# skhu101/HumanLiff

Measured on AMD Instinct MI355X. Metric: denoise-steps/sec, higher is better.
Workload: dtype f32; 1 GPU; configs[1]: 256x256x27 tri-plane UNet (controlnet, 497M params), 1000-step DDPM p_sample_loop, batch=4 per GPU; global_batch=4, parallelism=replicas x1 (subjects sharded, final all-gather only)

## Files before the change

### humanliff_amd/_lib.py

```python
import contextlib
import ctypes as C
import os

import torch

_HERE = os.path.dirname(os.path.abspath(__file__))
LIB_PATH = os.environ.get("HL_LIB_PATH") or os.path.join(_HERE, "libhumanliff_hip.so")

HL_RENDER_MLP_FP16 = 16
HL_RENDER_MLP_BF16X3 = 32
HL_RENDER_MLP_FP16X2 = 64
HL_RENDER_FOUR_LAUNCH = 128
HL_CONV_FP32 = 0
HL_CONV_BF16X3 = 1
HL_CONV_FP32_F23 = 3
HL_CONV_FP32_DIRECT = 2
HL_CONV_BF16 = 4
HL_CONV_FP16 = 5
HL_CONV_FP32_MFMA = 6
HL_RENDER_WHITE_BKGD = 1
HL_RENDER_NORMALIZE_DEPTH = 2
HL_RENDER_REEVALUATE = 4
HL_RENDER_CLAMP_DEPTH = 8
HL_COMPOSITE_SERIAL_RAW = 1
# ... 74 lines not shown
    "hl_render_composite_backward_plan": (_i, [_i, _i]),
    "hl_render_mlp_bwd_packed_bytes": (_sz, []),
    "hl_render_mlp_pack_bwd": (_i, [C.POINTER(RenderMlpParams), _p, _p]),
    "hl_render_train_rows": (None, [C.POINTER(C.c_int), C.POINTER(C.c_int)]),
    "hl_render_eval_acts": (_i, [_p, _p, _i, _i, _p, _p, _p, _p, _p, _p, _i, _i64, _i, _p, _p, _i64, _i64, _p]),
    "hl_render_composite_backward_scratch_bytes": (_sz, [_i64, _i, _i]),
    "hl_render_composite_backward": (_i, [_p, _p, _p, _p, _p, _p, _p, _p, _p, _i64, _i, _i, _u, _p, _p, _p, _i64, _p, _p]),
    "hl_render_eval_points_acts": (_i, [_p, _p, _i, _i, _p, _p, _p, _i64, _i, _p, _p, _i64, _i64, _p]),
    "hl_render_plane_grads_points_scratch_bytes": (_sz, [_i64, _i, _i]),
    "hl_render_plane_grads_points": (_i, [_i, _i, _p, _p, _p, _i64, _i, _i, _p, _i64, _p, _p, _p]),
    "hl_render_weight_grads": (_i, [_p, _i64, _p, _i64, _i64, C.POINTER(RenderMlpParams), _p, _p]),
    "hl_render_weight_grads_scratch_bytes": (_sz, [_i64]),
    "hl_render_plane_grads_scratch_bytes": (_sz, [_i64]),
    "hl_render_mlp_backward": (_i, [_p, _p, _i, _i, _p, _p, _p, _p, _p, _p, _i, _i64, _i, _p, _p, _i64, _i64, _p, _i64, _i64, _p]),
    "hl_render_plane_grads": (_i, [_i, _i, _p, _p, _p, _p, _p, _p, _p, _i, _i64, _i, _i, _p, _i64, _p, _p, _p]),
    "hl_render_fine": (_i, [_p, _p, _i, _i, _p, _p, _p, _p, _p, _p, _i, _i64, _i, _u, _p, _p, _p, _p]),
    "hl_unet_packed_bytes": (_sz, [C.POINTER(UNetCfg)]),
    "hl_unet_create": (_i, [C.POINTER(UNetCfg), _i, C.POINTER(C.c_char_p), C.POINTER(C.c_void_p), C.POINTER(C.c_int64),
                            _p, _p, C.POINTER(C.c_void_p)]),
    "hl_unet_destroy": (None, [_p]),
    "hl_unet_workspace_bytes": (_sz, [_p, _i, _i, _i]),
    "hl_unet_forward": (_i, [_p, _p, _p, _p, _p, _p, _p, _i, _i, _i, _p, _p]),
    "hl_unet_set_overlap": (_i, [_p, _i]),
    "hl_unet_set_conv_mode": (_i, [_p, _i]),
    "hl_unet_profile": (_i, [_p, _i]),
    "hl_unet_profile_read": (_i, [_p, C.POINTER(C.c_double), C.POINTER(C.c_double), C.POINTER(C.c_int64)]),
    "hl_unet_profile_read_ex": (_i, [_p, C.POINTER(C.c_double), C.POINTER(C.c_double), C.POINTER(C.c_double), C.POINTER(C.c_int64)]),
    "hl_unet_dispatch_census": (_i, [_p, C.POINTER(C.c_int64)]),
    "hl_unet_dispatch_census_ex": (_i, [_p, _p, _i]),
    "hl_unet_profile_dominant": (_i, [_p, C.POINTER(C.c_double), C.POINTER(C.c_int)]),
    "hl_diffusion_step": (_i, [_i, _p, _p, _p, _p, _p, _p, _p, _i64, _i, _i, _i, _p, _p]),
    "hl_diffusion_q_sample": (_i, [_p, _p, _p, _p, _p, _i64, _i, _i, _p]),
    "hl_diffusion_reverse_step": (_i, [_i, _p, _p, _p, _p, _p, _p, _i64, _i, _i, _i, _p]),
    "hl_diffusion_vb_scratch_bytes": (_sz, [_i64, _i]),
    "hl_diffusion_vb_terms": (_i, [_i, _i, _i, _p, _p, _p, _p, _p, _i64, _p, _p, _i64, _i, _i, _p, _p, _p, _i64, _i64, _p, _sz, _p]),
    "hl_diffusion_prior_bpd": (_i, [_p, _p, _i64, _i, _i, _p, _p, _sz, _p]),
    "hl_conv2d_scratch_bytes": (_sz, [_i] * 10),
    "hl_conv2d_plan": (_i, [_i] * 10 + [C.POINTER(C.c_int), C.POINTER(C.c_int)]),
    "hl_conv2d_plan_ex": (_i, [_i] * 12 + [C.POINTER(C.c_int)]),
    "hl_conv2d_gn_scratch_bytes": (_sz, [_i] * 10),
    "hl_conv2d_bwd_data_scratch_bytes": (_sz, [_i] * 11),
    "hl_conv2d_nhwc": (_i, [_p, _i, _i, _i, _i, _p, _p, _i, _i, _i, _i, _p, _p, _i, _p, _p, _p, _sz, _p]),
    "hl_conv2d_nhwc_mode": (_i, [_i, _p, _i, _i, _i, _i, _p, _p, _i, _i, _i, _i, _p, _p, _i, _p, _p, _p, _sz, _p]),
    "hl_conv2d_nhwc_gn": (_i, [_i, _p, _i, _i, _i, _i, _p, _p, _i, _i, _i, _i, _p, _p, _i, _p, _p, _p, _p, _p, _p, C.POINTER(C.c_int), _p, _sz, _p]),
    "hl_conv2d_bwd_data_plan": (_i, [_i] * 11 + [C.POINTER(C.c_int), C.POINTER(C.c_int)]),
    "hl_conv2d_nhwc_bwd_data": (_i, [_i, _p, _i, _i, _i, _i, _p, _i, _i, _i, _i, _i, _p, _i, _p, _sz, _p]),
# ... 165 lines not shown
```

### humanliff_amd/csrc/hl_unet.cpp

```cpp
#include <cstdint>
#include <string>
#include <unordered_map>
#include <utility>
#include <vector>

#include "hl_stat_book.h"
#include "hl_unet_kernels.h"
#include <algorithm>

namespace {

using hl::ConvArgs;
using hl::View;

static inline int round_up(int v, int m) { return (v + m - 1) / m * m; }

using hl::WeightForm;
using hl::conv_forms;
using hl::conv_mode_known;

struct Conv {
    hl::ConvWeights w;
    const float *bias = nullptr;
    int Cin = 0, Cin_pad = 0, Cout = 0, ks = 1;
};
struct Norm {
    const float *gamma = nullptr, *beta = nullptr;
    int C = 0;
    float eps = 1e-5f;
};
struct Res {
    Norm n1, n2;
    Conv c1, c2, skip;
    bool has_skip = false;
    bool aware = false;
    long emb_off = 0;
    int Cin = 0, Cout = 0;
};
struct Attn {
    Norm norm;
    Conv qkv, proj;
    int C = 0, heads = 1;
};
struct Xf {
    Norm norm;
    Conv proj_in, proj_out, qkv, out1, ff_in, ff_out;
    const float *ln1_g = nullptr, *ln1_b = nullptr, *ln3_g = nullptr, *ln3_b = nullptr;
    const float *v2_w = nullptr, *o2_w = nullptr, *o2_b = nullptr;
    int C = 0, heads = 1;
};
enum Kind { K_CONV, K_RES, K_ATTN, K_DOWN, K_UP, K_XF };
struct Layer {
    Kind kind;
    int idx;
};
struct Block {
    std::vector<Layer> layers;
    int Cout = 0;
    int ds_out = 1;
};

struct Net {
    hl_unet_cfg cfg{};
    std::unordered_map<std::string, std::pair<const float *, int64_t>> sd;
    std::vector<Conv> convs;
    std::vector<Res> res;
    std::vector<Attn> attn;
    std::vector<Xf> xf;
    std::vector<Block> in_blocks, out_blocks, cond_blocks;
    Block middle;
    std::vector<int> proj_cond;
    Conv out_conv;
    Norm out_norm;
    const float *te0_w = nullptr, *te0_b = nullptr, *te2_w = nullptr, *te2_b = nullptr, *label = nullptr;
    Conv ada1, ada2;
    const float *ada_w = nullptr, *ada_b = nullptr;
    const float *emb_w = nullptr, *emb_b = nullptr;
    long emb_total = 0;
    int E = 0;
    int Cpad0 = 0;
    float *packed = nullptr;
    size_t packed_off = 0;
    bool dry = true;
    hipStream_t st = nullptr;
    std::string err;
    hipStream_t side = nullptr;
    hipEvent_t ev_fork = nullptr, ev_join = nullptr;
    std::vector<hipEvent_t> ev_block;
    bool overlap = true;
    int conv_mode = HL_CONV_FP32;
    bool prof = false;
    std::vector<hipEvent_t> ev_pool;
    struct Span { int cat; size_t a, b; double flops, exec; int key[5]; long mid; };
    double dom[4] = {0, 0, 0, 0};
// ... 26 lines not shown
    if (expect >= 0 && it->second.second != expect) {
        if (n.err.empty()) n.err = "shape mismatch for " + name + ": got " + std::to_string(it->second.second) + " elements, expected " + std::to_string(expect);
        return nullptr;
    }
    return it->second.first;
}

size_t form_floats(size_t bytes) { return (bytes / 4 + 63) / 64 * 64; }
size_t conv_forms_floats(int Cout, int Cin_pad, int ks) {
    size_t t = 0;
    for (int f = 0; f < hl::kWeightForms; ++f) t += form_floats(hl::conv_form_bytes((WeightForm)f, Cout, Cin_pad, ks));
    return t;
}
Conv make_conv_w(Net &n, const float *w, const float *bias, int Cin, int Cout, int ks, bool ups = false);
Conv make_conv(Net &n, const std::string &p, int Cin, int Cout, int ks, bool has_bias = true, bool ups = false) {
    const float *w = lookup(n, p + ".weight", (int64_t)Cout * Cin * ks * ks);
    const float *b = has_bias ? lookup(n, p + ".bias", Cout) : nullptr;
    return make_conv_w(n, w, b, Cin, Cout, ks, ups);
}
Conv make_conv_w(Net &n, const float *w, const float *bias, int Cin, int Cout, int ks, bool ups) {
    Conv c;
    c.Cin = Cin; c.Cin_pad = round_up(Cin, 16); c.Cout = Cout; c.ks = ks;
    c.bias = n.dry ? nullptr : bias;
    const int cp = c.Cin_pad;
    for (int f = 0; f < hl::kWeightForms; ++f) {
        const size_t bytes = hl::conv_form_bytes((WeightForm)f, Cout, cp, ks, true, ups);
        if (!bytes) continue;
        float *dst = n.dry ? nullptr : n.packed + n.packed_off;
        n.packed_off += form_floats(bytes);
        if (n.dry || !w) continue;
        c.w.p[f] = dst;
        if (hl::conv_pack_form((WeightForm)f, w, Cout, Cin, cp, ks, dst, n.st) != 0 && n.err.empty()) n.err = hl_last_error();
    }
    return c;
}
Norm make_norm(Net &n, const std::string &p, int C) {
    Norm g;
    g.C = C;
    g.gamma = lookup(n, p + ".weight", C);
    g.beta = lookup(n, p + ".bias", C);
    return g;
}

struct EmbPiece { std::string name; int O; long off; };

int add_res(Net &n, std::vector<EmbPiece> &emb, const std::string &p, int Cin, int Cout, bool aware = false) {
// ... 92 lines not shown
            ch = co;
            if (has_ds(c, ds)) {
                if (c.cross_attn) b.layers.push_back({K_XF, add_xf(n, p + ".1", ch, c.num_heads)});
                else b.layers.push_back({K_ATTN, add_attn(n, p + ".1", ch, c.num_heads)});
            }
            b.Cout = ch; b.ds_out = ds;
            blocks.push_back(b);
            chans.push_back(ch);
            ++bi;
        }
        if (level != c.n_levels - 1) {
            Block b;
            const std::string p = root + "." + std::to_string(bi);
            b.layers.push_back({K_DOWN, add_conv(n, p + ".0.op", ch, ch, 3)});
            ds *= 2;
            b.Cout = ch; b.ds_out = ds;
            blocks.push_back(b);
            chans.push_back(ch);
            ++bi;
        }
    }
}

void build(Net &n) {
    const hl_unet_cfg &c = n.cfg;
    n.E = 4 * c.model_channels;
    n.Cpad0 = round_up(c.in_channels, 16);
    n.emb_total = 0;
    n.packed_off = 0;
    n.convs.clear(); n.res.clear(); n.attn.clear(); n.xf.clear();
    n.in_blocks.clear(); n.out_blocks.clear(); n.cond_blocks.clear(); n.proj_cond.clear();
    std::vector<EmbPiece> emb;
    n.te0_w = lookup(n, "time_embed.0.weight", (int64_t)n.E * c.model_channels);
    n.te0_b = lookup(n, "time_embed.0.bias", n.E);
    n.te2_w = lookup(n, "time_embed.2.weight", (int64_t)n.E * n.E);
    n.te2_b = lookup(n, "time_embed.2.bias", n.E);
    n.label = c.num_classes > 0 ? lookup(n, "label_emb.weight", (int64_t)c.num_classes * n.E) : nullptr;
    if (c.adagn || c.cross_attn) {
        n.ada1 = make_conv(n, "conv_proj_1", c.out_channels, 6, 3);
        n.ada2 = make_conv(n, "conv_proj_2", 6, 1, 3);
        n.ada_w = lookup(n, "linear.weight", (int64_t)n.E * 4096);
        n.ada_b = lookup(n, "linear.bias", n.E);
    }

    std::vector<int> chans;
    const bool aware = c.aware3d != 0;
// ... 21 lines not shown
            int li = 0;
            b.layers.push_back({K_RES, add_res(n, emb, p + "." + std::to_string(li++), ch + skip, co, aware)});
            ch = co;
            if (has_ds(c, ds)) {
                if (c.cross_attn) b.layers.push_back({K_XF, add_xf(n, p + "." + std::to_string(li++), ch, c.num_heads)});
                else b.layers.push_back({K_ATTN, add_attn(n, p + "." + std::to_string(li++), ch, c.num_heads_upsample)});
            }
            if (level && i == c.num_res_blocks) {
                b.layers.push_back({K_UP, add_conv(n, p + "." + std::to_string(li++) + ".conv", ch, ch, 3, true)});
                ds /= 2;
            }
            b.Cout = ch; b.ds_out = ds;
            n.out_blocks.push_back(b);
            ++bi;
        }
    }
    n.out_norm = make_norm(n, "out.0", ch);
    n.out_conv = make_conv(n, "out.2", c.model_channels, c.out_channels, 3);
    if (c.controlnet) {
        std::vector<int> cch;
        build_encoder(n, emb, "input_blocks_cond", n.cond_blocks, cch, false);
        for (size_t i = 0; i < n.cond_blocks.size(); ++i)
            n.proj_cond.push_back(add_conv(n, "input_blocks_proj_cond." + std::to_string(i), cch[i], cch[i], 1));
    }
    const size_t wfl = (size_t)n.emb_total * n.E;
    if (!n.dry) {
        float *wdst = n.packed + n.packed_off, *bdst = wdst + wfl;
        for (auto &e : emb) {
            const float *w = lookup(n, e.name + ".weight", (int64_t)e.O * n.E);
            const float *b = lookup(n, e.name + ".bias", e.O);
            if (!w || !b) continue;
            hipMemcpyAsync(wdst + (size_t)e.off * n.E, w, (size_t)e.O * n.E * sizeof(float), hipMemcpyDeviceToDevice, n.st);
            hipMemcpyAsync(bdst + e.off, b, (size_t)e.O * sizeof(float), hipMemcpyDeviceToDevice, n.st);
        }
        n.emb_w = wdst; n.emb_b = bdst;
    }
    n.packed_off += (wfl + n.emb_total + 63) / 64 * 64;
}

struct Aff { float *cA = nullptr, *cB = nullptr; hl::GnSrc gn{}; };
struct ConvOpt {
    int stride = 1, ups = 0;
    Aff af{};
    int act = 0;
    const float *res = nullptr; long res_pitch = 0;
    float *out2 = nullptr; long out2_pitch = 0;
// ... 109 lines not shown
        n.census[hl::conv_census_row(pl.path)][lvl] += 1;
        span_key[0] = (int)pl.path; span_key[1] = lvl; span_key[2] = o.ups ? 1 : 0; span_key[3] = c.Cout; span_key[4] = c.ks;
        const double fl = 2.0 * (double)out.pixels() * c.Cout * c.Cin * c.ks * c.ks;
        span_end(CAT_CONV, e0, fl, fl * hl::conv_issued_factor(pl.path) * (pl.kernel == hl::ConvKernel::H2sUp ? 4.0 / 9.0 : 1.0));
    }
    Aff coef(const View &x, const Norm &g, const float *emb, bool force_arrays = false) {
        Aff af;
        af.cA = alloc((size_t)B * x.C);
        af.cB = alloc((size_t)B * x.C);
        if (!run) return af;
        const float *gt = book.totals_of(x.p, x.C, true);
        if (gt && !force_arrays && !n.prof) {
            af.cA = af.cB = nullptr;
            af.gn.gt = gt; af.gn.C = x.C; af.gn.HW = x.H * x.W;
            af.gn.gamma = g.gamma; af.gn.beta = g.beta; af.gn.emb = emb; af.gn.emb_pitch = n.emb_total; af.gn.eps = g.eps;
            return af;
        }
        const size_t e0 = span_begin();
        if (gt) ok(hl::groupnorm_coef_stats(x, gt, g.gamma, g.beta, emb, n.emb_total, af.cA, af.cB, lane->st, g.eps));
        else ok(hl::groupnorm_coef(x, g.gamma, g.beta, emb, n.emb_total, af.cA, af.cB, lane->gn_scratch, lane->st, nullptr, g.eps));
        span_end(CAT_GN, e0, 0.0);
        return af;
    }
    void res_block(const Res &r, const View &x, const View &dst) {
        const bool noss = n.cfg.no_scale_shift;
        ConvOpt o1, o2;
        o1.af = coef(x, r.n1, nullptr); o1.act = 1; o1.stats = !noss;
        View h = plain(H / dst.H, r.Cout), in2 = h;
        conv(r.c1, x, h, o1);
        if (noss && run) ok(hl::add_rowvec(h, emb_all + r.emb_off, lane->st, n.emb_total));
        const Aff a2 = coef(h, r.n2, run && !noss ? emb_all + r.emb_off : nullptr, r.aware);
        if (r.aware) {
            in2 = plain(H / dst.H, 3 * r.Cout);
            float *sums = alloc((size_t)B * 3 * (h.H + h.W / 3) * r.Cout);
            if (run) {
                const size_t e0 = span_begin();
                ok(hl::gn_apply_3d(h, a2.cA, a2.cB, sums, in2.p, lane->st));
                span_end(CAT_GN, e0, 0.0);
            }
        } else {
            o2.af = a2; o2.act = 1;
        }
        if (r.has_skip) {
            ConvOpt sk;
            sk.stats = false;
            conv(r.skip, x, dst, sk);
        }
        o2.residual(r.has_skip ? dst : x);
        conv(r.c2, in2, dst, o2);
    }
    void attn_block(const Attn &a, const View &x, const View &dst) {
        ConvOpt oq, op;
        oq.af = coef(x, a.norm, nullptr);
        oq.stats = false;
        View qkv = plain(H / x.H, 3 * a.C);
        conv(a.qkv, x, qkv, oq);
        View o = plain(H / x.H, a.C);
        float *ost = alloc_stat(hl::conv_stats_floats(B, (long)x.H * x.W));
        if (run) {
            const size_t e0 = span_begin();
            int emitted = 0;
            ok(hl::attention(qkv.p, B, x.H * x.W, a.C, a.heads, o.p, lane->st, n.conv_mode == HL_CONV_FP32, ost, &emitted));
            if (emitted) book.produced(o.p, {ost, a.C, 0}, a.C); else book.stored_without_totals(o.p);
            const double T = (double)x.H * x.W;
            span_end(CAT_ATTN, e0, 4.0 * B * T * T * a.C);
        }
        op.residual(x);
        conv(a.proj, o, dst, op);
    }
    void xf_block(const Xf &a, const View &x, const View &dst) {
        const int ds = H / x.H;
        hipStream_t st = lane->st;
// ... 126 lines not shown
                if (run && c.controlnet) book.concat_halves(cat[j].p, cat[j].C, ch, cat_st);
                ch = n.out_blocks[j].Cout;
            }
        }
        auto first_part = [&](size_t j, int C) { View v = cat[j]; v.C = C; return v; };
        const bool fork = run && c.controlnet && n.overlap && !n.prof && n.side;
        if (fork) {
            hipEventRecord(n.ev_fork, st);
            hipStreamWaitEvent(n.side, n.ev_fork, 0);
        }
        std::vector<View> hs(nb);
        View h = xin;
        for (size_t i = 0; i < nb; ++i) {
            hs[i] = plain(n.in_blocks[i].ds_out, n.in_blocks[i].Cout);
            block(n.in_blocks[i], h, hs[i]);
            if (fork) hipEventRecord(n.ev_block[i], st);
            h = hs[i];
        }
        block(n.middle, h, first_part(0, n.middle.Cout));
        if (c.controlnet) {
            if (fork) lane = &lanes[1];
            View hc = xsum;
            for (size_t i = 0; i < nb; ++i) {
                View tmp = plain(n.cond_blocks[i].ds_out, n.cond_blocks[i].Cout);
                block(n.cond_blocks[i], hc, tmp);
                View pj = plain(n.cond_blocks[i].ds_out, n.cond_blocks[i].Cout);
                const size_t j = nb - 1 - i;
                const int Ch = cat[j].C - hs[i].C;
                if (fork) hipStreamWaitEvent(n.side, n.ev_block[i], 0);
                ConvOpt zo;
                zo.out2 = run ? cat[j].p + Ch : nullptr; zo.out2_pitch = cat[j].pitch; zo.res2 = hs[i].p; zo.res2_pitch = hs[i].pitch;
                conv(n.convs[n.proj_cond[i]], tmp, pj, zo);
                hc = pj;
            }
            if (fork) {
                hipEventRecord(n.ev_join, n.side);
                lane = &lanes[0];
                hipStreamWaitEvent(st, n.ev_join, 0);
            }
        } else if (run) {
            for (size_t i = 0; i < nb; ++i) {
                const size_t j = nb - 1 - i;
                const int Ch = cat[j].C - hs[i].C;
                hipMemcpy2DAsync(cat[j].p + Ch, cat[j].pitch * sizeof(float), hs[i].p, hs[i].pitch * sizeof(float),
                                 (size_t)hs[i].C * sizeof(float), (size_t)hs[i].pixels(), hipMemcpyDeviceToDevice, st);
                book.stored_without_totals(cat[j].p + Ch);
            }
        }
        View last;
        for (size_t j = 0; j < nb; ++j) {
            View dst = (j + 1 < nb) ? first_part(j + 1, n.out_blocks[j].Cout) : plain(n.out_blocks[j].ds_out, n.out_blocks[j].Cout);
            block(n.out_blocks[j], cat[j], dst);
            last = dst;
        }
        ConvOpt oo;
// ... 61 lines not shown
        return rc;
    }
    if (n->cfg.controlnet) {
        bool okc = hipStreamCreateWithFlags(&n->side, hipStreamNonBlocking) == hipSuccess;
        okc = okc && hipEventCreateWithFlags(&n->ev_fork, hipEventDisableTiming) == hipSuccess;
        okc = okc && hipEventCreateWithFlags(&n->ev_join, hipEventDisableTiming) == hipSuccess;
        n->ev_block.assign(n->in_blocks.size(), nullptr);
        for (auto &e : n->ev_block) okc = okc && hipEventCreateWithFlags(&e, hipEventDisableTiming) == hipSuccess;
        if (!okc) {
            (void)hipGetLastError();
            if (n->side) { hipStreamDestroy(n->side); n->side = nullptr; }
        }
    }
    *handle = n;
    return HL_OK;
}

int hl_unet_set_overlap(void *handle, int enable) {
    HL_REQUIRE(handle, "hl_unet_set_overlap: null handle");
    static_cast<Net *>(handle)->overlap = enable != 0;
    return HL_OK;
}

int hl_unet_set_conv_mode(void *handle, int mode) {
    HL_REQUIRE(handle, "hl_unet_set_conv_mode: null handle");
    HL_REQUIRE(conv_mode_known(mode), "hl_unet_set_conv_mode: unknown mode %d", mode);
    static_cast<Net *>(handle)->conv_mode = mode;
    return HL_OK;
}

void hl_unet_destroy(void *handle) { delete static_cast<Net *>(handle); }

size_t hl_unet_workspace_bytes(void *handle, int B, int H, int W) {
    if (!handle || B <= 0) return 0;
    Net &n = *static_cast<Net *>(handle);
    Exec e(n, false, nullptr, nullptr, B, H, n.cfg.aware3d ? 3 * W : W);
    e.forward(nullptr, nullptr, nullptr, nullptr, nullptr, nullptr);
    WsLayout L;
    return ws_layout(e.off, e.act_need, e.stat_off, 0, &L) ? 0 : L.total;
}

int hl_unet_forward(void *handle, const float *x, const int64_t *t, const float *t_float, const float *x_cond,
                    const int64_t *y, float *out, int B, int H, int W, void *workspace, void *stream) {
    HL_REQUIRE(handle && x && (t || t_float) && out && workspace, "hl_unet_forward: null argument");
    Net &n = *static_cast<Net *>(handle);
    const int total_ds = 1 << (n.cfg.n_levels - 1);
    HL_REQUIRE(B >= 1 && B <= 16, "hl_unet_forward: batch %d outside [1,16]", B);
    HL_REQUIRE(H % total_ds == 0 && W % total_ds == 0, "hl_unet_forward: H,W must be divisible by %d", total_ds);
    HL_REQUIRE(!n.cfg.controlnet || x_cond, "hl_unet_forward: x_cond is required with cond_type='controlnet'");
    HL_REQUIRE(!(n.cfg.adagn || n.cfg.cross_attn) || (x_cond && H == 256 && W == 256),
               "hl_unet_forward: cond_type='AdaGN' / 'cross_attention' need x_cond and 256x256 inputs (Linear(64*64, ..))");
    HL_REQUIRE(n.cfg.num_classes == 0 || y, "hl_unet_forward: y is required for a class-conditional model");
    if (n.cfg.aware3d) W *= 3;
    Exec dry(n, false, nullptr, nullptr, B, H, W);
    dry.forward(nullptr, nullptr, nullptr, nullptr, nullptr, nullptr);
    char *const ws = static_cast<char *>(workspace);
    WsLayout L;
    const int lrc = ws_layout(dry.off, dry.act_need, dry.stat_off, reinterpret_cast<uintptr_t>(ws), &L);
    if (lrc) return lrc;
    Exec e(n, true, ws, (hipStream_t)stream, B, H, W);
// ... 332 lines not shown
    View v; v.p = out; v.N = N; conv_out_hw(H, W, ks, stride, upsample, &v.H, &v.W); v.C = Cout; v.pitch = Cout;
    if (h_used_stats) *h_used_stats = slots;
    if (slots > 0) {
        return hl::groupnorm_coef_stats(v, stats, gamma, beta, nullptr, 0, next_coefA, next_coefB, (hipStream_t)stream);
    }
    return hl::groupnorm_coef(v, gamma, beta, nullptr, 0, next_coefA, next_coefB, gn_scr, (hipStream_t)stream);
}

int hl_conv2d_nhwc(const float *in, int N, int H, int W, int Cin, const float *w_oihw, const float *bias, int Cout, int ks,
                   int stride, int upsample, const float *coefA, const float *coefB, int silu, const float *residual,
                   float *out, void *scratch, size_t scratch_bytes, void *stream) {
    return conv2d_single(HL_CONV_FP32_DIRECT, in, N, H, W, Cin, w_oihw, bias, Cout, ks, stride, upsample, coefA, coefB, silu, residual, out,
                         scratch, scratch_bytes, stream);
}

int hl_conv2d_nhwc_mode(int conv_mode, const float *in, int N, int H, int W, int Cin, const float *w_oihw, const float *bias,
                        int Cout, int ks, int stride, int upsample, const float *coefA, const float *coefB, int silu,
                        const float *residual, float *out, void *scratch, size_t scratch_bytes, void *stream) {
    HL_REQUIRE(conv_mode_known(conv_mode), "hl_conv2d_nhwc_mode: unknown mode %d", conv_mode);
    return conv2d_single(conv_mode, in, N, H, W, Cin, w_oihw, bias, Cout, ks, stride, upsample, coefA, coefB, silu, residual, out,
                         scratch, scratch_bytes, stream);
}

int hl_debug_set_h16_min_blocks(long v) { hl::set_h16_min_blocks(v); return HL_OK; }
int hl_debug_set_single_op_scale_source(int from_totals) { g_single_op_scale_from_totals = from_totals != 0; return HL_OK; }
int hl_debug_set_attention_tiling(int query_tiles, int placement) { return hl::debug_set_attention_tiling(query_tiles, placement); }

size_t hl_groupnorm_scratch_bytes(int N) { return hl::gn_scratch_floats(N) * sizeof(float); }

int hl_groupnorm_coef(const float *x, int N, int H, int W, int C, const float *gamma, const float *beta, const float *emb,
                      float *coefA, float *coefB, void *scratch, size_t scratch_bytes, void *stream) {
    HL_REQUIRE(scratch && scratch_bytes >= hl_groupnorm_scratch_bytes(N), "hl_groupnorm_coef: scratch too small (%zu bytes, hl_groupnorm_scratch_bytes says %zu)",
               scratch_bytes, hl_groupnorm_scratch_bytes(N));
    View v; v.p = const_cast<float *>(x); v.N = N; v.H = H; v.W = W; v.C = C; v.pitch = C;
    return hl::groupnorm_coef(v, gamma, beta, emb, 2L * C, coefA, coefB, static_cast<float *>(scratch), (hipStream_t)stream);
}

int hl_timestep_embedding(const int64_t *t, const float *t_float, int B, int dim, float *out, void *stream) {
    HL_REQUIRE(dim % 2 == 0, "hl_timestep_embedding: odd dim %d", dim);
    return hl::timestep_embedding(t, t_float, B, dim, out, (hipStream_t)stream);
}

int hl_attention_nhwc(const float *qkv, int N, int T, int C, int heads, float *out, void *stream) {
    return hl::attention(qkv, N, T, C, heads, out, (hipStream_t)stream);
}

// ... 13 lines not shown
```

### humanliff_amd/csrc/hl_unet_kernels.h

```cpp
#pragma once
#include "hl_common.h"

namespace hl {

struct View {
    float *p = nullptr;
    int N = 0, H = 0, W = 0, C = 0;
    long pitch = 0;
    long pixels() const { return (long)N * H * W; }
};

struct GnSrc {
    const float *gt;
    int C, HW;
    const float *gamma, *beta, *emb;
    long emb_pitch;
    float eps;
};

enum class ConvPath : int {
    Direct = 0,
    Wino2 = 1,
    Bf16x3 = 2,
    Wino4 = 3,
// ... 5 lines not shown
}
constexpr double conv_issued_factor(ConvPath p) {
    return p == ConvPath::Wino2 ? 16.0 / 36.0 : (p == ConvPath::Wino4 ? 0.25 : (p == ConvPath::Bf16x3 ? 6.0 : 1.0));
}

enum class WeightForm : int {
    Fp32,
    Bf16x3,
    Wino2,
    Wino4,
    Fp16x2,
    H16,
    Fp16x2Up,
    kCount
};
constexpr int kWeightForms = (int)WeightForm::kCount;
constexpr unsigned form_bit(WeightForm f) { return 1u << (int)f; }
constexpr WeightForm form_of(ConvPath p) {
    return p == ConvPath::Wino2 ? WeightForm::Wino2 : p == ConvPath::Bf16x3 ? WeightForm::Bf16x3 : p == ConvPath::Wino4 ? WeightForm::Wino4 :
           p == ConvPath::H16 ? WeightForm::H16 : p == ConvPath::Fp16x2 ? WeightForm::Fp16x2 : WeightForm::Fp32;
}
size_t conv_form_bytes(WeightForm f, int Cout, int Cin_pad, int ks, bool cap_wino4 = true, bool ups = false);
int conv_pack_form(WeightForm f, const float *w, int Cout, int Cin, int Cin_pad, int ks, void *dst, hipStream_t st, int tf = 0, int f16 = 1);
const float *conv_h2_wscale(const void *packed, int Cout, int Cin_pad, int ks);
const float *conv_h2p_wscale(const void *packed, int Cout, int Cin_pad);

struct ConvWeights {
    const void *p[kWeightForms] = {};
    bool has(WeightForm f) const { return p[(int)f] != nullptr; }
    const float *fp32() const { return static_cast<const float *>(p[(int)WeightForm::Fp32]); }
    ConvWeights only(unsigned mask) const {
        ConvWeights r;
        for (int f = 0; f < kWeightForms; ++f) if (mask >> f & 1u) r.p[f] = p[f];
        return r;
    }
};

constexpr bool conv_mode_known(int mode) {
    return mode == HL_CONV_FP32 || mode == HL_CONV_FP32_MFMA || mode == HL_CONV_BF16X3 || mode == HL_CONV_FP32_DIRECT || mode == HL_CONV_FP32_F23 ||
           mode == HL_CONV_BF16 || mode == HL_CONV_FP16;
}
constexpr bool conv_mode_bf16(int mode) { return mode == HL_CONV_BF16X3 || mode == HL_CONV_BF16; }
constexpr unsigned conv_forms(int mode, bool bf16_h16, bool bwd_data) {
    const bool f32 = mode == HL_CONV_FP32 || mode == HL_CONV_FP32_MFMA || mode == HL_CONV_FP16;
    return form_bit(WeightForm::Fp32) | (conv_mode_bf16(mode) ? form_bit(WeightForm::Bf16x3) : 0u) |
           (f32 || mode == HL_CONV_FP32_F23 ? form_bit(WeightForm::Wino2) : 0u) | (f32 ? form_bit(WeightForm::Wino4) : 0u) |
// ... 128 lines not shown
```

### humanliff_amd/csrc/hl_unet_kernels.hip

```cpp
#include "hl_unet_kernels.h"

#include <algorithm>
#include <cstdlib>
#include <type_traits>

#include "hl_reduce.h"
#include "hl_stats.h"
#include "hl_xcd_map.h"

namespace hl {
namespace {

__device__ __forceinline__ float silu_f(float v) { return v * __builtin_amdgcn_rcpf(1.f + __builtin_amdgcn_exp2f(-1.44269504088896341f * v)); }

constexpr int KG = 4;
__host__ __device__ inline void kt_decode(int kt, int ncc, int taps, int &cc, int &tap) {
    const int per = KG * taps;
    const int cg = kt / per, r = kt - cg * per;
    const int g = (ncc - cg * KG) < KG ? (ncc - cg * KG) : KG;
    tap = r / g;
    cc = cg * KG + (r - tap * g);
}


// ... 1666 lines not shown
                           n < p.Cout, (long)p.Hout * p.Wout, s, q);
        }
    }
}

__global__ void k_pack_conv(const float *__restrict__ w, int Cout, int Cin, int Cin_pad, int ks, int rows, float *__restrict__ dst, int tf) {
    const int taps = ks * ks;
    const long Ktot = (long)Cin_pad * taps;
    const long n = (long)rows * Ktot;
    for (long i = (long)blockIdx.x * blockDim.x + threadIdx.x; i < n; i += (long)gridDim.x * blockDim.x) {
        const int o = (int)(i / Ktot);
        const long k = i - (long)o * Ktot;
        const int c16 = (int)(k & 15);
        const long t = k >> 4;
        int cc, tap;
        kt_decode((int)t, Cin_pad >> 4, taps, cc, tap);
        const int cin = cc * 16 + c16;
        float v = 0.f;
        if (o < Cout && cin < Cin) v = tf ? w[((long)cin * Cout + o) * taps + (taps - 1 - tap)] : w[((long)o * Cin + cin) * taps + tap];
        dst[i] = v;
    }
}

__global__ void k_pack_conv_bf3(const float *__restrict__ w, int Cout, int Cin, int Cin_pad, int ks, int rows,
                                unsigned short *__restrict__ dst, int tf) {
    const int taps = ks * ks;
    const long Ktot = (long)Cin_pad * taps;
    const long n = (long)rows * Ktot;
    for (long i = (long)blockIdx.x * blockDim.x + threadIdx.x; i < n; i += (long)gridDim.x * blockDim.x) {
        const int o = (int)(i / Ktot);
        const long k = i - (long)o * Ktot;
        const int c16 = (int)(k & 15);
        const long t = k >> 4;
        int cc, tap;
        kt_decode((int)t, Cin_pad >> 4, taps, cc, tap);
        const int cin = cc * 16 + c16;
        float v = 0.f;
        if (o < Cout && cin < Cin) v = tf ? w[((long)cin * Cout + o) * taps + (taps - 1 - tap)] : w[((long)o * Cin + cin) * taps + tap];
        const unsigned uh = __float_as_uint(v) & 0xffff0000u;
        const float r1 = v - __uint_as_float(uh);
        const unsigned um = __float_as_uint(r1) & 0xffff0000u;
        const float r2 = r1 - __uint_as_float(um);
        const unsigned ul = __float_as_uint(r2);
        unsigned short *q = dst + ((long)o * (Ktot >> 4) + t) * 48 + (c16 >> 3) * 8 + (c16 & 7);
        q[0] = (unsigned short)(uh >> 16);
        q[16] = (unsigned short)(um >> 16);
// ... 893 lines not shown

int conv_pack_form(WeightForm f, const float *w, int Cout, int Cin, int Cin_pad, int ks, void *dst, hipStream_t st, int tf, int f16) {
    HL_REQUIRE(w && dst && Cin <= Cin_pad && (ks == 1 || ks == 3) && (f > WeightForm::Bf16x3 || Cin_pad % 16 == 0) &&
                   conv_form_bytes(f, Cout, Cin_pad, ks, false, f == WeightForm::Fp16x2Up),
               "conv_pack_form: bad argument (form %d)", (int)f);
    const int rows = round_up(Cout, 64);
    float *dstf = static_cast<float *>(dst);
    switch (f) {
    case WeightForm::Fp32: hipLaunchKernelGGL(k_pack_conv, dim3(1024), dim3(256), 0, st, w, Cout, Cin, Cin_pad, ks, rows, dstf, tf); break;
    case WeightForm::Bf16x3: hipLaunchKernelGGL(k_pack_conv_bf3, dim3(1024), dim3(256), 0, st, w, Cout, Cin, Cin_pad, ks, rows, static_cast<unsigned short *>(dst), tf); break;
    case WeightForm::Wino2:
        hipLaunchKernelGGL(k_pack_conv_wino, dim3((unsigned)std::min<long>(8192, (long)(Cout >> 5) * (Cin_pad >> 3))), dim3(256), 0, st, w, Cout, Cin, Cin_pad, dstf, tf);
        break;
    case WeightForm::Wino4:
        hipLaunchKernelGGL(k_pack_conv_wino4, dim3((unsigned)std::min<long>(8192, (long)(round_up(Cout, 32) >> 5) * (Cin_pad >> 3))), dim3(256), 0, st, w, Cout, Cin, Cin_pad, dstf, tf);
        break;
    case WeightForm::Fp16x2: return conv_pack_weights_h2(w, Cout, Cin, Cin_pad, ks, dst, st, tf);
    case WeightForm::Fp16x2Up: return conv_pack_weights_h2p(w, Cout, Cin, Cin_pad, ks, dst, st, tf);
    default: return conv_pack_weights_h16(w, Cout, Cin, Cin_pad, ks, dst, f16, st, tf);
    }
    return check_launch("k_pack_conv");
}

constexpr long kH16MinBlocks = 48;
static long g_h16_min_blocks = -1;
static long h16_min_blocks() { return g_h16_min_blocks >= 0 ? g_h16_min_blocks : kH16MinBlocks; }
void set_h16_min_blocks(long v) { g_h16_min_blocks = v; }

struct SplitK { int splits, kt_per; };
static SplitK split_k(const ConvArgs &a, int nk, int want, long blocks = 0, long min_blocks = 0) {
    const long M = (long)a.out.N * a.out.H * a.out.W;
    if (!a.splitk_ws) want = 1;
    while (want > 1 && (size_t)want * M * a.Cout * sizeof(float) > a.splitk_ws_bytes) --want;
    if (want < 2 || blocks * want < min_blocks) return {1, nk};
    const int kt = (nk + want - 1) / want;
    return {(nk + kt - 1) / kt, kt};
}

ConvPlan plan_conv(const ConvArgs &a) {
    ConvPlan pl;
    const bool gn_on = a.coefA != nullptr || a.gn.gt != nullptr;
    const bool bf16 = conv_mode_bf16(a.mode);
    const bool h2 = a.w.has(WeightForm::Fp16x2) && !bf16;
    pl.gn_mode = gn_on ? (a.act ? 2 : 1) : 0;
    const long M = (long)a.out.N * a.out.H * a.out.W, hw_o = (long)a.out.H * a.out.W;
    const int cpad = round_up(a.Cout, 64);
// ... 42 lines not shown
            return done(a.stats, (int)(hw_o / 128));
        }
    }
    constexpr long h2_min_blocks = 12;
    const long h2_blocks = (M / 256) * (a.Cout / 192);
    if (h2 && (!gn_on || a.act_ws) && !a.out_nchw && conv1_h2_applies(a.out.H, a.out.W, a.in.C, a.Cout, a.ks, a.stride, a.ups) &&
        in_31 && a.in.pitch % 4 == 0 && h2_blocks >= h2_min_blocks) {
        constexpr long h2_split_max = 64;
        const int nk48 = a.in.C / 48;
        take(ConvPath::Fp16x2, ConvKernel::H2s1,
             split_k(a, nk48, h2_blocks < h2_split_max && !a.out2 ? (int)std::min<long>(std::min<long>(128 / std::max<long>(h2_blocks, 1), nk48 / 4), 8) : 1));
        const bool fuse1 = a.in.C <= 4096;
        if (gn_on && !fuse1) pl.pre = ConvPrePass::Dense;
        return done(a.stats, 1);
    }
    constexpr long h3_min_blocks = 100;
    if (h2 && a.ks == 3 && (!gn_on || (a.act_ws && !a.ups)) && !a.out_nchw &&
        conv_h16_applies(a.out.H, a.out.W, a.in.C, a.Cout, a.ks, a.stride, a.ups) && in_31 && a.in.pitch % 4 == 0) {
        constexpr long h3_split_min = 8;
        constexpr long h3_min_chunks = 2;
        constexpr long h3_max_splits = 16;
        constexpr long h3_target = 256;
        const bool fills = h16_blocks >= h3_min_blocks;
        const int want = h16_blocks >= h3_split_min && !a.out2 ? (int)std::min<long>(std::min<long>(h3_target / h16_blocks, nk32 / h3_min_chunks), h3_max_splits) : 0;
        const SplitK sk = split_k(a, nk32, fills ? 1 : want);
        if (fills || sk.splits > 1) {
            const bool phases = a.w.has(WeightForm::Fp16x2Up) && conv3_h2s_ph_applies(a.out.H, a.out.W, a.in.C, a.Cout, a.ks, a.stride, a.ups);
            take(ConvPath::Fp16x2, phases ? ConvKernel::H2sUp : ConvKernel::H2s, sk);
            const bool fuse = !a.ups && a.in.C <= 4096;
            if (gn_on && !fuse) pl.pre = ConvPrePass::TwoPlane;
            return done(a.stats, (int)(hw_o / 128));
        }
    }
    constexpr long h3d_min_blocks = 32;
    if (h2 && a.ks == 3 && a.stride == 2 && !a.ups && !gn_on && !a.out_nchw && conv3_h2d_applies(a.out.H, a.out.W, a.in.C, a.Cout) &&
        in_31 && a.in.pitch % 4 == 0 && h16_blocks >= h3d_min_blocks) {
        take(ConvPath::Fp16x2, ConvKernel::H2d, {1, direct_sk.kt_per});
        return done(a.stats, (int)(hw_o / 128));
    }

    const ConvPrePass dense = gn_on ? ConvPrePass::Dense : ConvPrePass::None;
    const int nk8 = a.in.C / 8;
    constexpr long wino4_thr = 512;
    const bool small_nchw = a.out_nchw && a.Cout < 32 && !a.res && !a.out2 && !a.stats && (!gn_on || a.act_ws) && in_31;
    const long wino4_blocks = (long)a.out.N * (a.out.H / 16) * (a.out.W / 32) * ((a.Cout + 31) / 32);
    if ((dma || small_nchw) && a.w.has(WeightForm::Wino4) && !bf16 && a.ks == 3 && a.stride == 1 && a.out.H % 16 == 0 && a.out.W % 32 == 0 &&
        (a.Cout % 32 == 0 || small_nchw) && (long)round_up(a.Cout, 32) * a.in.C * 144 < (1L << 31)) {
// ... 437 lines not shown
```

### humanliff_amd/improved_diffusion/unet.py

```python
import ctypes as C

import torch as th
import torch.nn as nn

from .. import _lib
from .nn import SiLU, conv_nd, linear, normalization, zero_module


class TimestepBlock(nn.Module):
    pass


class TimestepEmbedSequential(nn.Sequential, TimestepBlock):
    pass


class Upsample(nn.Module):
    def __init__(self, channels, use_conv, dims=2):
        super().__init__()
        assert use_conv, "conv_resample=False is not built"
        self.channels, self.use_conv, self.dims = channels, use_conv, dims
        self.conv = conv_nd(dims, channels, channels, 3, padding=1)


# ... 225 lines not shown
            L.hl_unet_destroy(self._hip[0])
            self._hip = None
        dev = None
        for k, v in sd.items():
            if not v.is_cuda:
                raise RuntimeError("UNetModel parameters must be on the GPU (model.to('cuda')); there is no CPU path")
            if v.dtype != th.float32 or not v.is_contiguous():
                raise RuntimeError(f"parameter {k} must be contiguous fp32")
            dev = v.device
        cfg = self._cfg()
        nbytes = L.hl_unet_packed_bytes(C.byref(cfg))
        if nbytes == 0:
            _lib.check(-1, "hl_unet_packed_bytes")
        packed = th.empty(nbytes // 4 + 64, dtype=th.float32, device=dev)
        n = len(sd)
        names = (C.c_char_p * n)(*[k.encode() for k in sd])
        ptrs = (C.c_void_p * n)(*[v.data_ptr() for v in sd.values()])
        numels = (C.c_int64 * n)(*[v.numel() for v in sd.values()])
        handle = C.c_void_p()
        with th.cuda.device(dev):
            _lib.check(L.hl_unet_create(C.byref(cfg), n, names, ptrs, numels, _lib.ptr(packed), _lib.stream_ptr(),
                                        C.byref(handle)), "hl_unet_create")
        _lib.check(L.hl_unet_set_conv_mode(handle, self._conv_mode), "hl_unet_set_conv_mode")
        self._hip = (handle, packed, key)
        self._ws = {}
        return handle

    def set_conv_mode(self, mode):
        modes = {"fp32": _lib.HL_CONV_FP32, "fp32_mfma": _lib.HL_CONV_FP32_MFMA, "bf16x3": _lib.HL_CONV_BF16X3, "fp32_direct": _lib.HL_CONV_FP32_DIRECT, "fp32_f23": _lib.HL_CONV_FP32_F23,
                 "fp16": _lib.HL_CONV_FP16}
        if mode not in modes:
            raise ValueError(f"unknown conv mode {mode!r} (expected one of {sorted(modes)})")
        self._conv_mode = modes[mode]
        if self._hip is not None:
            _lib.check(_lib.lib().hl_unet_set_conv_mode(self._hip[0], self._conv_mode), "hl_unet_set_conv_mode")
        return self

    def dispatch_census(self):
        if self._hip is None:
            raise RuntimeError("dispatch_census: no forward has run yet")
        counts = (C.c_int64 * 40)()
        _lib.check(_lib.lib().hl_unet_dispatch_census_ex(self._hip[0], counts, 5), "hl_unet_dispatch_census_ex")
        return {name: [int(counts[p * 8 + l]) for l in range(8)] for p, name in enumerate(("direct", "wino2", "bf16x3", "wino4", "fp16x2"))}

    def __del__(self):
        try:
            if self._hip is not None:
                _lib.lib().hl_unet_destroy(self._hip[0])
        except Exception:
# ... 52 lines not shown
```

### include/humanliff_hip.h

```cpp
#ifndef HUMANLIFF_HIP_H
#define HUMANLIFF_HIP_H

#include <stddef.h>
#include <stdint.h>

#ifdef __cplusplus
extern "C" {
#endif

typedef enum hl_status {
    HL_OK = 0,
    HL_ERR_INVALID = -1,
    HL_ERR_UNSUPPORTED = -2,
    HL_ERR_RUNTIME = -3
} hl_status;

int hl_version(void);
const char *hl_last_error(void);


typedef struct hl_render_mlp_params {
    const float *pts0_w, *pts0_b;
    const float *pts1_w, *pts1_b;
    const float *pts2_w, *pts2_b;
// ... 131 lines not shown
    int n_attention_ds;
    int attention_ds[8];
    int num_heads, num_heads_upsample;
    int num_classes;
    int controlnet;
    int adagn;
    int cross_attn;
    int aware3d;
    int no_scale_shift;
} hl_unet_cfg;

size_t hl_unet_packed_bytes(const hl_unet_cfg *cfg);

int hl_unet_create(const hl_unet_cfg *cfg, int n_tensors, const char *const *names, const void *const *ptrs,
                   const int64_t *numels, void *packed, void *stream, void **handle);
void hl_unet_destroy(void *handle);

size_t hl_unet_workspace_bytes(void *handle, int B, int H, int W);

int hl_unet_forward(void *handle, const float *x, const int64_t *t, const float *t_float, const float *x_cond,
                    const int64_t *y, float *out, int B, int H, int W, void *workspace, void *stream);

int hl_unet_set_overlap(void *handle, int enable);

#define HL_CONV_FP32 0
#define HL_CONV_BF16X3 1
#define HL_CONV_FP32_DIRECT 2
#define HL_CONV_FP32_F23 3
#define HL_CONV_BF16 4
#define HL_CONV_FP16 5
#define HL_CONV_FP32_MFMA 6
int hl_unet_set_conv_mode(void *handle, int mode);

int hl_unet_profile(void *handle, int enable);
int hl_unet_profile_read(void *handle, double *h_ms, double *h_flops, int64_t *h_launches);
int hl_unet_profile_read_ex(void *handle, double *h_ms, double *h_flops, double *h_exec_flops, int64_t *h_launches);

int hl_unet_profile_dominant(void *handle, double *h_vals, int *h_key);

int hl_unet_dispatch_census(void *handle, int64_t *h_counts);
int hl_unet_dispatch_census_ex(void *handle, int64_t *h_counts, int rows);

int hl_diffusion_step(int mode, const float *x, const float *eps, const float *noise, const float *coef,
                      const int64_t *t, float *sample, float *pred_xstart, int64_t n_per_sample, int B, int T, int clip,
                      const float *log_variance, void *stream);

// ... 280 lines not shown
```

Measured before the change: 155.6 denoise-steps/s.

## Fold ControlNet zero-conv projections into preceding conv weights at build time

At model creation, each ControlNet condition block's 1x1 zero-conv projection is composed with the block's last conv (and its skip conv) into a single convolution, computed on device in double precision. The forward pass then runs the folded conv directly, writing the projected output and residual. This removes one 1x1 conv launch and one intermediate activation per condition block. It also lets split-K run for convs that write a second output, and it adds packed-weight storage for the composed forms, with small numerical differences from reassociating the maths.

```diff
diff --git a/humanliff_amd/_lib.py b/humanliff_amd/_lib.py
--- a/humanliff_amd/_lib.py
+++ b/humanliff_amd/_lib.py
@@ -120,6 +120,8 @@
     "hl_unet_workspace_bytes": (_sz, [_p, _i, _i, _i]),
     "hl_unet_forward": (_i, [_p, _p, _p, _p, _p, _p, _p, _i, _i, _i, _p, _p]),
     "hl_unet_set_overlap": (_i, [_p, _i]),
+    "hl_unet_set_fold_zero_convs": (_i, [_p, _i]),
+    "hl_conv_compose_zero": (_i, [_p, _p, _p, _p, _i, _i, _i, _i, _p, _p, _p]),
     "hl_unet_set_conv_mode": (_i, [_p, _i]),
     "hl_unet_profile": (_i, [_p, _i]),
     "hl_unet_profile_read": (_i, [_p, C.POINTER(C.c_double), C.POINTER(C.c_double), C.POINTER(C.c_int64)]),
diff --git a/humanliff_amd/csrc/hl_unet.cpp b/humanliff_amd/csrc/hl_unet.cpp
--- a/humanliff_amd/csrc/hl_unet.cpp
+++ b/humanliff_amd/csrc/hl_unet.cpp
@@ -22,6 +22,7 @@
 struct Conv {
     hl::ConvWeights w;
     const float *bias = nullptr;
+    const float *w_src = nullptr;
     int Cin = 0, Cin_pad = 0, Cout = 0, ks = 1;
 };
 struct Norm {
@@ -49,6 +50,10 @@
     const float *v2_w = nullptr, *o2_w = nullptr, *o2_b = nullptr;
     int C = 0, heads = 1;
 };
+struct Fold {
+    bool on = false;
+    Conv last, skip;
+};
 enum Kind { K_CONV, K_RES, K_ATTN, K_DOWN, K_UP, K_XF };
 struct Layer {
     Kind kind;
@@ -70,6 +75,8 @@
     std::vector<Block> in_blocks, out_blocks, cond_blocks;
     Block middle;
     std::vector<int> proj_cond;
+    std::vector<Fold> fold_cond;
+    bool fold = true;
     Conv out_conv;
     Norm out_norm;
     const float *te0_w = nullptr, *te0_b = nullptr, *te2_w = nullptr, *te2_b = nullptr, *label = nullptr;
@@ -142,6 +149,7 @@
     Conv c;
     c.Cin = Cin; c.Cin_pad = round_up(Cin, 16); c.Cout = Cout; c.ks = ks;
     c.bias = n.dry ? nullptr : bias;
+    c.w_src = n.dry ? nullptr : w;
     const int cp = c.Cin_pad;
     for (int f = 0; f < hl::kWeightForms; ++f) {
         const size_t bytes = hl::conv_form_bytes((WeightForm)f, Cout, cp, ks, true, ups);
@@ -280,6 +288,52 @@
     }
 }
 
+Conv fold_conv(Net &n, const Conv &z, const Conv &c, bool add_bz, float *stage) {
+    float *bc = n.dry ? nullptr : n.packed + n.packed_off;
+    n.packed_off += form_floats((size_t)z.Cout * sizeof(float));
+    if (!n.dry && z.w_src && c.w_src &&
+        hl::compose_zero_conv(z.w_src, add_bz ? z.bias : nullptr, c.w_src, c.bias, z.Cout, c.Cout, c.Cin, c.ks * c.ks, stage, bc, n.st) != 0 && n.err.empty())
+        n.err = hl_last_error();
+    return make_conv_w(n, n.dry ? reinterpret_cast<const float *>(16) : (z.w_src && c.w_src ? stage : nullptr), bc, c.Cin, z.Cout, c.ks);
+}
+void build_folds(Net &n) {
+    const size_t nb = n.cond_blocks.size();
+    n.fold_cond.assign(nb, Fold{});
+    auto last_conv = [&](const Block &b, const Conv **skip) -> const Conv * {
+        *skip = nullptr;
+        if (b.layers.size() != 1) return nullptr;
+        const Layer &L = b.layers[0];
+        if (L.kind == K_CONV || L.kind == K_DOWN) return &n.convs[L.idx];
+        if (L.kind != K_RES || !n.res[L.idx].has_skip || n.res[L.idx].aware) return nullptr;
+        *skip = &n.res[L.idx].skip;
+        return &n.res[L.idx].c2;
+    };
+    size_t stage_floats = 0;
+    for (size_t i = 0; i < nb; ++i) {
+        const Conv *sk, *c = last_conv(n.cond_blocks[i], &sk);
+        if (!c) continue;
+        stage_floats = std::max(stage_floats, (size_t)c->Cout * c->Cin * c->ks * c->ks);
+        if (sk) stage_floats = std::max(stage_floats, (size_t)sk->Cout * sk->Cin * (n.dry ? 9 : sk->ks * sk->ks));
+    }
+    float *stage = n.dry ? nullptr : n.packed + n.packed_off;
+    n.packed_off += form_floats(stage_floats * sizeof(float));
+    for (size_t i = 0; i < nb; ++i) {
+        const Conv *sk, *c = last_conv(n.cond_blocks[i], &sk);
+        if (!c) continue;
+        const Conv z = n.convs[n.proj_cond[i]];
+        Fold &f = n.fold_cond[i];
+        f.on = true;
+        f.last = fold_conv(n, z, *c, true, stage);
+        if (sk) {
+            f.skip = fold_conv(n, z, *sk, false, stage);
+            if (n.dry) {
+                const size_t f1 = conv_forms_floats(z.Cout, sk->Cin_pad, 1), f3 = conv_forms_floats(z.Cout, sk->Cin_pad, 3);
+                if (f3 > f1) n.packed_off += f3 - f1;
+            }
+        }
+    }
+}
+
 void build(Net &n) {
     const hl_unet_cfg &c = n.cfg;
     n.E = 4 * c.model_channels;
@@ -347,6 +401,7 @@
         build_encoder(n, emb, "input_blocks_cond", n.cond_blocks, cch, false);
         for (size_t i = 0; i < n.cond_blocks.size(); ++i)
             n.proj_cond.push_back(add_conv(n, "input_blocks_proj_cond." + std::to_string(i), cch[i], cch[i], 1));
+        build_folds(n);
     }
     const size_t wfl = (size_t)n.emb_total * n.E;
     if (!n.dry) {
@@ -502,9 +557,9 @@
         span_end(CAT_GN, e0, 0.0);
         return af;
     }
-    void res_block(const Res &r, const View &x, const View &dst) {
+    void res_block(const Res &r, const View &x, const View &dst, const Fold *fold = nullptr, const ConvOpt &tail = {}, hipEvent_t wait = nullptr) {
         const bool noss = n.cfg.no_scale_shift;
-        ConvOpt o1, o2;
+        ConvOpt o1, o2 = tail;
         o1.af = coef(x, r.n1, nullptr); o1.act = 1; o1.stats = !noss;
         View h = plain(H / dst.H, r.Cout), in2 = h;
         conv(r.c1, x, h, o1);
@@ -524,10 +579,11 @@
         if (r.has_skip) {
             ConvOpt sk;
             sk.stats = false;
-            conv(r.skip, x, dst, sk);
+            conv(fold ? fold->skip : r.skip, x, dst, sk);
         }
         o2.residual(r.has_skip ? dst : x);
-        conv(r.c2, in2, dst, o2);
+        if (wait) hipStreamWaitEvent(lane->st, wait, 0);
+        conv(fold ? fold->last : r.c2, in2, dst, o2);
     }
     void attn_block(const Attn &a, const View &x, const View &dst) {
         ConvOpt oq, op;
@@ -700,15 +756,31 @@
             if (fork) lane = &lanes[1];
             View hc = xsum;
             for (size_t i = 0; i < nb; ++i) {
-                View tmp = plain(n.cond_blocks[i].ds_out, n.cond_blocks[i].Cout);
-                block(n.cond_blocks[i], hc, tmp);
-                View pj = plain(n.cond_blocks[i].ds_out, n.cond_blocks[i].Cout);
+                const Block &cb = n.cond_blocks[i];
+                const Fold *fold = n.fold && n.fold_cond[i].on ? &n.fold_cond[i] : nullptr;
                 const size_t j = nb - 1 - i;
                 const int Ch = cat[j].C - hs[i].C;
-                if (fork) hipStreamWaitEvent(n.side, n.ev_block[i], 0);
                 ConvOpt zo;
                 zo.out2 = run ? cat[j].p + Ch : nullptr; zo.out2_pitch = cat[j].pitch; zo.res2 = hs[i].p; zo.res2_pitch = hs[i].pitch;
-                conv(n.convs[n.proj_cond[i]], tmp, pj, zo);
+                View pj;
+                if (fold) {
+                    pj = plain(cb.ds_out, cb.Cout);
+                    const Layer &L = cb.layers[0];
+                    hipEvent_t wait = fork ? n.ev_block[i] : nullptr;
+                    if (L.kind == K_RES) {
+                        res_block(n.res[L.idx], hc, pj, fold, zo, wait);
+                    } else {
+                        if (L.kind == K_DOWN) zo.stride = 2;
+                        if (wait) hipStreamWaitEvent(n.side, wait, 0);
+                        conv(fold->last, hc, pj, zo);
+                    }
+                } else {
+                    View tmp = plain(cb.ds_out, cb.Cout);
+                    block(cb, hc, tmp);
+                    pj = plain(cb.ds_out, cb.Cout);
+                    if (fork) hipStreamWaitEvent(n.side, n.ev_block[i], 0);
+                    conv(n.convs[n.proj_cond[i]], tmp, pj, zo);
+                }
                 hc = pj;
             }
             if (fork) {
@@ -816,6 +888,12 @@
     return HL_OK;
 }
 
+int hl_unet_set_fold_zero_convs(void *handle, int enable) {
+    HL_REQUIRE(handle, "hl_unet_set_fold_zero_convs: null handle");
+    static_cast<Net *>(handle)->fold = enable != 0;
+    return HL_OK;
+}
+
 int hl_unet_set_conv_mode(void *handle, int mode) {
     HL_REQUIRE(handle, "hl_unet_set_conv_mode: null handle");
     HL_REQUIRE(conv_mode_known(mode), "hl_unet_set_conv_mode: unknown mode %d", mode);
@@ -828,8 +906,11 @@
 size_t hl_unet_workspace_bytes(void *handle, int B, int H, int W) {
     if (!handle || B <= 0) return 0;
     Net &n = *static_cast<Net *>(handle);
+    const bool fold = n.fold;
+    n.fold = false;
     Exec e(n, false, nullptr, nullptr, B, H, n.cfg.aware3d ? 3 * W : W);
     e.forward(nullptr, nullptr, nullptr, nullptr, nullptr, nullptr);
+    n.fold = fold;
     WsLayout L;
     return ws_layout(e.off, e.act_need, e.stat_off, 0, &L) ? 0 : L.total;
 }
@@ -1208,6 +1289,11 @@
                          scratch, scratch_bytes, stream);
 }
 
+int hl_conv_compose_zero(const float *wz, const float *bz, const float *w, const float *b, int Cout, int Cmid, int Cin, int ks, float *wc, float *bc, void *stream) {
+    HL_REQUIRE(ks == 1 || ks == 3, "hl_conv_compose_zero: kernel size %d", ks);
+    return hl::compose_zero_conv(wz, bz, w, b, Cout, Cmid, Cin, ks * ks, wc, bc, (hipStream_t)stream);
+}
+
 int hl_debug_set_h16_min_blocks(long v) { hl::set_h16_min_blocks(v); return HL_OK; }
 int hl_debug_set_single_op_scale_source(int from_totals) { g_single_op_scale_from_totals = from_totals != 0; return HL_OK; }
 int hl_debug_set_attention_tiling(int query_tiles, int placement) { return hl::debug_set_attention_tiling(query_tiles, placement); }
diff --git a/humanliff_amd/csrc/hl_unet_kernels.h b/humanliff_amd/csrc/hl_unet_kernels.h
--- a/humanliff_amd/csrc/hl_unet_kernels.h
+++ b/humanliff_amd/csrc/hl_unet_kernels.h
@@ -51,6 +51,7 @@
 }
 size_t conv_form_bytes(WeightForm f, int Cout, int Cin_pad, int ks, bool cap_wino4 = true, bool ups = false);
 int conv_pack_form(WeightForm f, const float *w, int Cout, int Cin, int Cin_pad, int ks, void *dst, hipStream_t st, int tf = 0, int f16 = 1);
+int compose_zero_conv(const float *wz, const float *bz, const float *w, const float *b, int Cout, int Cmid, int Cin, int taps, float *wc, float *bc, hipStream_t st);
 const float *conv_h2_wscale(const void *packed, int Cout, int Cin_pad, int ks);
 const float *conv_h2p_wscale(const void *packed, int Cout, int Cin_pad);
 
diff --git a/humanliff_amd/csrc/hl_unet_kernels.hip b/humanliff_amd/csrc/hl_unet_kernels.hip
--- a/humanliff_amd/csrc/hl_unet_kernels.hip
+++ b/humanliff_amd/csrc/hl_unet_kernels.hip
@@ -1712,6 +1712,30 @@
     }
 }
 
+constexpr int kComposeRows = 8;
+__global__ __launch_bounds__(256) void k_compose_zero_conv(const float *__restrict__ wz, const float *__restrict__ bz, const float *__restrict__ w,
+                                                           const float *__restrict__ b, int Cout, int Cmid, long K, float *__restrict__ wc, float *__restrict__ bc) {
+    const long j = (long)blockIdx.x * 256 + threadIdx.x;
+    const int o0 = blockIdx.y * kComposeRows;
+    if (j > K) return;
+    const bool is_b = j == K;
+    double acc[kComposeRows];
+#pragma unroll
+    for (int r = 0; r < kComposeRows; ++r) acc[r] = 0.0;
+    for (int m = 0; m < Cmid; ++m) {
+        const double x = is_b ? (b ? (double)b[m] : 0.0) : (double)w[(long)m * K + j];
+#pragma unroll
+        for (int r = 0; r < kComposeRows; ++r) acc[r] += (double)wz[(long)min(o0 + r, Cout - 1) * Cmid + m] * x;
+    }
+#pragma unroll
+    for (int r = 0; r < kComposeRows; ++r) {
+        const int o = o0 + r;
+        if (o >= Cout) break;
+        if (is_b) bc[o] = (float)(acc[r] + (bz ? (double)bz[o] : 0.0));
+        else wc[(long)o * K + j] = (float)acc[r];
+    }
+}
+
 __global__ void k_pack_conv_bf3(const float *__restrict__ w, int Cout, int Cin, int Cin_pad, int ks, int rows,
                                 unsigned short *__restrict__ dst, int tf) {
     const int taps = ks * ks;
@@ -2651,6 +2675,14 @@
     return check_launch("k_pack_conv");
 }
 
+int compose_zero_conv(const float *wz, const float *bz, const float *w, const float *b, int Cout, int Cmid, int Cin, int taps, float *wc, float *bc, hipStream_t st) {
+    HL_REQUIRE(wz && w && wc && bc && Cout > 0 && Cmid > 0 && Cin > 0 && (taps == 1 || taps == 9), "compose_zero_conv: bad argument");
+    const long K = (long)Cin * taps;
+    hipLaunchKernelGGL(k_compose_zero_conv, dim3((unsigned)((K + 1 + 255) / 256), (unsigned)((Cout + kComposeRows - 1) / kComposeRows)), dim3(256), 0, st,
+                       wz, bz, w, b, Cout, Cmid, K, wc, bc);
+    return check_launch("k_compose_zero_conv");
+}
+
 constexpr long kH16MinBlocks = 48;
 static long g_h16_min_blocks = -1;
 static long h16_min_blocks() { return g_h16_min_blocks >= 0 ? g_h16_min_blocks : kH16MinBlocks; }
@@ -2739,7 +2771,7 @@
         constexpr long h3_max_splits = 16;
         constexpr long h3_target = 256;
         const bool fills = h16_blocks >= h3_min_blocks;
-        const int want = h16_blocks >= h3_split_min && !a.out2 ? (int)std::min<long>(std::min<long>(h3_target / h16_blocks, nk32 / h3_min_chunks), h3_max_splits) : 0;
+        const int want = h16_blocks >= h3_split_min ? (int)std::min<long>(std::min<long>(h3_target / h16_blocks, nk32 / h3_min_chunks), h3_max_splits) : 0;
         const SplitK sk = split_k(a, nk32, fills ? 1 : want);
         if (fills || sk.splits > 1) {
             const bool phases = a.w.has(WeightForm::Fp16x2Up) && conv3_h2s_ph_applies(a.out.H, a.out.W, a.in.C, a.Cout, a.ks, a.stride, a.ups);
diff --git a/humanliff_amd/improved_diffusion/unet.py b/humanliff_amd/improved_diffusion/unet.py
--- a/humanliff_amd/improved_diffusion/unet.py
+++ b/humanliff_amd/improved_diffusion/unet.py
@@ -271,9 +271,16 @@
             _lib.check(L.hl_unet_create(C.byref(cfg), n, names, ptrs, numels, _lib.ptr(packed), _lib.stream_ptr(),
                                         C.byref(handle)), "hl_unet_create")
         _lib.check(L.hl_unet_set_conv_mode(handle, self._conv_mode), "hl_unet_set_conv_mode")
+        _lib.check(L.hl_unet_set_fold_zero_convs(handle, int(getattr(self, "_fold_zero_convs", True))), "hl_unet_set_fold_zero_convs")
         self._hip = (handle, packed, key)
         self._ws = {}
         return handle
+
+    def set_fold_zero_convs(self, enable=True):
+        self._fold_zero_convs = bool(enable)
+        if self._hip is not None:
+            _lib.check(_lib.lib().hl_unet_set_fold_zero_convs(self._hip[0], int(self._fold_zero_convs)), "hl_unet_set_fold_zero_convs")
+        return self
 
     def set_conv_mode(self, mode):
         modes = {"fp32": _lib.HL_CONV_FP32, "fp32_mfma": _lib.HL_CONV_FP32_MFMA, "bf16x3": _lib.HL_CONV_BF16X3, "fp32_direct": _lib.HL_CONV_FP32_DIRECT, "fp32_f23": _lib.HL_CONV_FP32_F23,
diff --git a/include/humanliff_hip.h b/include/humanliff_hip.h
--- a/include/humanliff_hip.h
+++ b/include/humanliff_hip.h
@@ -177,6 +177,10 @@
                     const int64_t *y, float *out, int B, int H, int W, void *workspace, void *stream);
 
 int hl_unet_set_overlap(void *handle, int enable);
+
+int hl_unet_set_fold_zero_convs(void *handle, int enable);
+int hl_conv_compose_zero(const float *wz, const float *bz, const float *w, const float *b, int Cout, int Cmid, int Cin, int ks, float *wc, float *bc,
+                         void *stream);
 
 #define HL_CONV_FP32 0
 #define HL_CONV_BF16X3 1
```

Measured after the change: 157.1 denoise-steps/s, median of 6. Within noise of the previous version (+0.9%).
